# tum-pbs/PhiFlow

Measured on NVIDIA H100. Metric: smoke_plume_512^3_steps_per_sec, higher is better.
Workload: dtype f32

## Files before the change

phiflow_b200/csrc/cg_common.cuh:

```cuda
#pragma once
#include "phi_internal.cuh"

#define CG_MAX_BATCH 1024
#define CG_MAX_GRID 2048

struct CgArgs {
    DGrid g; DField pf; UnitMap um;
    const float* rhs; float* x; float* r; float* d0; float* d1;
    const float* acc;
    double* partials;
    PhiCgResult* result;
    PhiCgParams prm;
};

struct CgShared {
    double (*warp_acc)[32];
    double* sum0;
    double* sum1;
    double* delta;
    float* alpha;
    float* aprev;
    float* beta;
    float* offs;
    float* mean;
    float* tol_sq;
    float* rsq0;
    int* iters;
    int* any_cont;
    unsigned char *cont, *conv, *divg;
    float* bprev;
};

__host__ __device__ inline size_t cg_smem_bytes(int batch)
{
    const size_t b8 = ((size_t)batch + 1) / 2 * 2;
    return 2 * 32 * sizeof(double) + 3 * b8 * sizeof(double) + 8 * b8 * sizeof(float)
         + (b8 + 2) * sizeof(int) + 3 * (b8 + 16);
}

__host__ __device__ __forceinline__ CgShared cg_carve(unsigned char* base, int batch)
{
    const size_t b8 = ((size_t)batch + 1) / 2 * 2;
    CgShared sh;
    unsigned char* p = base;
    sh.warp_acc = reinterpret_cast<double (*)[32]>(p); p += 2 * 32 * sizeof(double);
    sh.sum0 = (double*)p; p += b8 * sizeof(double);
    sh.sum1 = (double*)p; p += b8 * sizeof(double);
    sh.delta = (double*)p; p += b8 * sizeof(double);
    sh.alpha = (float*)p; p += b8 * sizeof(float);
    sh.aprev = (float*)p; p += b8 * sizeof(float);
    sh.beta = (float*)p; p += b8 * sizeof(float);
    sh.offs = (float*)p; p += b8 * sizeof(float);
    sh.mean = (float*)p; p += b8 * sizeof(float);
    sh.tol_sq = (float*)p; p += b8 * sizeof(float);
    sh.rsq0 = (float*)p; p += b8 * sizeof(float);
    sh.iters = (int*)p; p += b8 * sizeof(int);
    sh.any_cont = (int*)p; p += 2 * sizeof(int);
    sh.cont = p; p += b8 + 16;
    sh.conv = p; p += b8;
    sh.divg = p; p += (b8 + 3) / 4 * 4;
    sh.bprev = (float*)p;
    return sh;
}


#ifndef CG_BLOCK_WARPS
#define CG_BLOCK_WARPS PHI_WARPS_PER_CTA
#endif

__device__ __forceinline__ void flush_partials(const CgShared& sh, double* partials, int region, int batch, int b, double a0, double a1)
{
    const int warp = threadIdx.x >> 5, lane = threadIdx.x & 31;
    a0 = warp_sum(a0); a1 = warp_sum(a1);
    if (lane == 0) { sh.warp_acc[0][warp] = a0; sh.warp_acc[1][warp] = a1; }
    __syncthreads();
    if (threadIdx.x == 0) {
        double s0 = 0, s1 = 0;
        for (int w = 0; w < (int)(blockDim.x >> 5); ++w) { s0 += sh.warp_acc[0][w]; s1 += sh.warp_acc[1][w]; }
        const size_t G = gridDim.x;
        partials[((size_t)(region * 2 + 0) * batch + b) * G + blockIdx.x] = s0;
        partials[((size_t)(region * 2 + 1) * batch + b) * G + blockIdx.x] = s1;
    }
    __syncthreads();
}

__device__ __forceinline__ void reduce_partials(const CgShared& sh, const double* partials, int region, int batch, int units_per_batch,
                                                const unsigned char* active)
{
    const int warp = threadIdx.x >> 5, lane = threadIdx.x & 31;
    const int G = gridDim.x;
    const int cnt = min(units_per_batch, G);
    for (int b = warp; b < batch; b += (int)(blockDim.x >> 5)) {
        if (active && !active[b]) continue;
        const int first = (int)(((long long)b * units_per_batch) % G);
        double s0 = 0, s1 = 0;
        for (int i = lane; i < cnt; i += 32) {
            int c = first + i; if (c >= G) c -= G;
            s0 += __ldcg(&partials[((size_t)(region * 2 + 0) * batch + b) * G + c]);
            s1 += __ldcg(&partials[((size_t)(region * 2 + 1) * batch + b) * G + c]);
        }
        s0 = warp_sum(s0); s1 = warp_sum(s1);
        if (lane == 0) { sh.sum0[b] = s0; sh.sum1[b] = s1; }
    }
    __syncthreads();
}


template <bool MASK>
__device__ __forceinline__ void cg_balance(const CgShared& sh, const PhiCgParams& prm, int b, double cells)
{
    if (MASK) { sh.mean[b] = (prm.balance_rhs && sh.sum1[b] > 0.0) ? (float)(sh.sum0[b] / sh.sum1[b]) : 0.f; sh.offs[b] = 0.f; }
    else { sh.mean[b] = prm.balance_rhs ? (float)(sh.sum0[b] / cells) : 0.f; sh.offs[b] = prm.matrix_offset * (float)sh.sum1[b]; }
}

template <bool MASK>
__device__ __forceinline__ float cg_projection_mean(const CgShared& sh, int b, double cells)
{
    return MASK ? (sh.sum1[b] > 0.0 ? (float)(sh.sum0[b] / sh.sum1[b]) : 0.f) : (float)(sh.sum0[b] / cells);
}

__device__ __forceinline__ bool cg_iteration_done(const CgShared& sh, const PhiCgParams& prm, int b, double rsq_new)
{
    sh.delta[b] = rsq_new;
    const int it = ++sh.iters[b];
    const float rsq = fabsf((float)rsq_new);
    const bool conv = rsq <= sh.tol_sq[b];
    const bool divg = !isfinite(rsq) || (rsq / sh.rsq0[b] > 1e5f && it >= 8);
    const bool cont = !conv && !divg && it < prm.max_iter;
    sh.conv[b] = conv; sh.divg[b] = divg; sh.cont[b] = cont ? 1 : 0;
    return cont;
}


__device__ __forceinline__ void cg_count_running(const CgShared& sh, int batch)
{
    __syncthreads();
    if (threadIdx.x == 0) { int any = 0; for (int b = 0; b < batch; ++b) any |= sh.cont[b]; *sh.any_cont = any; }
    __syncthreads();
}

__device__ __forceinline__ void cg_start(const CgShared& sh, const PhiCgParams& prm, int batch)
{
    for (int b = threadIdx.x; b < batch; b += blockDim.x) {
        const double d0 = sh.sum0[b], d0tol = sh.sum1[b];
        sh.delta[b] = d0;
        const float tol = fmaxf(prm.rtol * prm.rtol * (float)d0tol, prm.atol * prm.atol);
        sh.tol_sq[b] = tol; sh.rsq0[b] = (float)d0;
        const bool conv = (float)d0 <= tol;
        const bool divg = !isfinite((float)d0);
        sh.conv[b] = conv; sh.divg[b] = divg; sh.iters[b] = 0;
        sh.cont[b] = (!conv && !divg && prm.max_iter > 0) ? 1 : 0;
        sh.beta[b] = 0.f; sh.alpha[b] = 0.f; sh.aprev[b] = 0.f;
    }
    cg_count_running(sh, batch);
}

__device__ __forceinline__ void cg_write_result(const CgShared& sh, PhiCgResult* result, int batch, bool comm_ok)
{
    if (blockIdx.x != 0) return;
    for (int b = threadIdx.x; b < batch; b += blockDim.x) {
        PhiCgResult res;
        res.iterations = sh.iters[b]; res.converged = sh.conv[b]; res.diverged = comm_ok ? sh.divg[b] : -1;
        res.residual_sq = fabsf((float)sh.delta[b]); res.tol_sq = sh.tol_sq[b]; res.initial_residual_sq = sh.rsq0[b];
        result[b] = res;
    }
}
```

phiflow_b200/csrc/ring_kernels.cu:

```cuda
#include <cooperative_groups.h>
#include <type_traits>
#include "cg_common.cuh"
#include <cstdlib>
#include <cstring>
#include "launch.cuh"

namespace cg = cooperative_groups;

#define RING_CONSUMERS 256
#define RING_THREADS (RING_CONSUMERS + 32)
#define RING_MAX_STAGES 8
#define RING_G 4

struct RingCfg {
    int TY, R, pitch, nx4;
    int stage_floats;
    int ZC, nyt, nzc;
    int units_per_batch, total_units;
    int consumers;
    int groups;
    int shfl_ok;
    int split, Zm, split_t;
};

// ... 764 lines not shown
__device__ __forceinline__ bool comm_allreduce(const CommDev& cm, const CgShared& sh, int batch, unsigned long long seq)
{
    const int par = (int)(seq & 1ull);
    const size_t stride = 2 * (size_t)CG_MAX_BATCH;
    if (blockIdx.x == 0) {
        for (int q = 0; q < cm.n; ++q) {
            double* dst = cm.mbox[q] + ((size_t)par * PHI_MAX_RANKS + cm.rank) * stride;
            for (int b = threadIdx.x; b < batch; b += blockDim.x) { dst[b] = sh.sum0[b]; dst[CG_MAX_BATCH + b] = sh.sum1[b]; }
        }
        __threadfence_system();
        __syncthreads();
        if ((int)threadIdx.x < cm.n) st_release_sys(cm.flag[threadIdx.x] + par * PHI_MAX_RANKS + cm.rank, seq);
    }
    bool ok = true;
    if ((int)threadIdx.x < cm.n) {
        const unsigned long long* f = cm.flag[cm.rank] + par * PHI_MAX_RANKS + threadIdx.x;
        const long long t0 = clock64();
        while (ld_acquire_sys(f) < seq) {
            if (clock64() - t0 > 40000000000ll) { ok = false; break; }
        }
    }
    ok = __syncthreads_and(ok);
    const double* src = cm.mbox[cm.rank] + (size_t)par * PHI_MAX_RANKS * stride;
    for (int b = threadIdx.x; b < batch; b += blockDim.x) {
        double s0 = 0, s1 = 0;
        for (int q = 0; q < cm.n; ++q) {
            s0 += *(volatile const double*)(src + q * stride + b);
            s1 += *(volatile const double*)(src + q * stride + CG_MAX_BATCH + b);
        }
        sh.sum0[b] = s0; sh.sum1[b] = s1;
    }
    __syncthreads();
    return ok;
}

template <int DIM, class F>
__device__ __forceinline__ void ring_unit_cells(const RingCfg& cfg, const DGrid& g, const DField& pf, const ThreadGroups& tg,
                                                const RingUnit& u, F&& fn)
{
    if ((int)threadIdx.x >= cfg.consumers) return;
    long long plane_off = (long long)u.b * pf.sb + (long long)u.y0 * pf.sy + (DIM == 3 ? (long long)u.z0 * pf.sz : 0);
    for (int z = u.z0; z < u.z1; ++z, plane_off += pf.sz)
#pragma unroll
        for (int k = 0; k < RING_G; ++k) {
            if (tg.j[k] < 0 || u.y0 + tg.j[k] >= g.n[1]) continue;
            const int x0 = tg.eoff[k] - tg.j[k] * cfg.pitch;
            fn(plane_off + tg.goff[k], min(4, g.n[0] - x0));
        }
}

#define FUSED_GI 2
#define FUSED_GH 2
#define FUSED_TILE_BUFS 3

struct FusedGroups {
    int ti[FUSED_GI], th[FUSED_GH];
    int ei[FUSED_GI], eh[FUSED_GH];
    int gi[FUSED_GI];
    unsigned vi, vh;
};

__device__ __forceinline__ void fused_groups_init(FusedGroups& fg, const RingCfg& cfg, const DGrid& g, const DField& pf)
{
    const int lane = threadIdx.x & 31, nx = g.n[0], pitch = cfg.pitch, nx4 = cfg.nx4;
    auto edge = [&](int jj, int x0) -> int {
        const int row = jj * pitch;
        if (lane == 0) return x0 == 0 ? (pf.klo[0] == PHI_BC_PERIODIC ? row + nx - 1 : row) : row + x0 - 1;
        if (lane == 31) return x0 + 4 >= nx ? (pf.khi[0] == PHI_BC_PERIODIC ? row : row + nx - 1) : row + x0 + 4;
        return 0;
    };
    fg.vi = fg.vh = 0;
#pragma unroll
    for (int k = 0; k < FUSED_GI; ++k) {
        const int ge = threadIdx.x + k * cfg.consumers;
        const int j = ge / nx4, x0 = (ge - j * nx4) * 4;
        if (j < cfg.TY) fg.vi |= 1u << k;
        fg.ti[k] = (j + 1) * pitch + x0;
        fg.ei[k] = edge(j + 1, x0);
        fg.gi[k] = j * (int)pf.sy + x0;
    }
#pragma unroll
    for (int k = 0; k < FUSED_GH; ++k) {
        const int ge = threadIdx.x + k * cfg.consumers;
        const int h = ge / nx4, x0 = (ge - h * nx4) * 4;
        const int jj = h == 0 ? 0 : cfg.TY + 1;
        if (h < 2) fg.vh |= 1u << k;
        fg.th[k] = jj * pitch + x0;
        fg.eh[k] = edge(jj, x0);
    }
}

__device__ __forceinline__ void prod_fused_setup(ProdUnit& pu, const RingCfg& cfg, const DField& pf, const float* d, const float* dprev,
                                                 int b, int y0)
{
    const int lane = threadIdx.x & 31, TY = cfg.TY;
    const uint32_t row_bytes = (uint32_t)cfg.pitch * 4u;
    const bool mergeable = pf.sy == cfg.pitch;
    const int rows[2] = {TY + 4, TY + 2};
    const int ylo[2] = {y0 - 2, y0 - 1};
    const float* src[2] = {d, dprev};
    int cnt[2] = {0, 0};
    pu.hmask = pu.emask = 0;
#pragma unroll
    for (int it = 0; it < 4; ++it) {
        const int line = lane + 32 * it;
        pu.yoff[it] = 0; pu.base[it] = nullptr; pu.dsto[it] = 0; pu.nbytes[it] = row_bytes;
        int key = -1, yv = 0, first = 0;
#pragma unroll
        for (int arr = 0; arr < 2; ++arr) {
            if (key < 0 && line >= first && line < first + rows[arr] && src[arr]) {
                int yy = ylo[arr] + (line - first); float cv;
                phi_resolve(yy, pf, 1, cv);
                pu.yoff[it] = (long long)b * pf.sb + (long long)yy * pf.sy;
                pu.base[it] = src[arr];
                pu.dsto[it] = 4u * (uint32_t)(line * cfg.pitch);
                key = arr; yv = yy;
            }
            first += rows[arr];
        }
        cnt[0] += key == 0; cnt[1] += key == 1;
        if (prod_merge_lines(key, yv, mergeable, row_bytes, pu.nbytes[it])) {
            if (key == 0) pu.hmask |= 1u << it; else pu.emask |= 1u << it;
        }
    }
#pragma unroll
    for (int c = 0; c < 2; ++c)
#pragma unroll
        for (int o = 16; o > 0; o >>= 1) cnt[c] += __shfl_xor_sync(0xffffffffu, cnt[c], o);
    pu.tot_h = cnt[0]; pu.tot_e = cnt[1];
}

__device__ __forceinline__ float4 lds4(const float* s, int off) { return *reinterpret_cast<const float4*>(s + off); }
__device__ __forceinline__ float dot4(const float4& a, const float4& b) { return a.x * b.x + a.y * b.y + a.z * b.z + a.w * b.w; }

__device__ __forceinline__ float4 stencil7(const float4& c, float xl, float xr, const float4& ym, const float4& yp, const float4& zm, const float4& zp,
                                           float ix2, float iy2, float iz2, float cc)
{
    float4 q;
    q.x = fmaf(ix2, xl + c.y, fmaf(iy2, ym.x + yp.x, -cc * c.x));
    q.y = fmaf(ix2, c.x + c.z, fmaf(iy2, ym.y + yp.y, -cc * c.y));
    q.z = fmaf(ix2, c.y + c.w, fmaf(iy2, ym.z + yp.z, -cc * c.z));
    q.w = fmaf(ix2, c.z + xr, fmaf(iy2, ym.w + yp.w, -cc * c.w));
    q.x = fmaf(iz2, zm.x + zp.x, q.x);
    q.y = fmaf(iz2, zm.y + zp.y, q.y);
    q.z = fmaf(iz2, zm.z + zp.z, q.z);
    q.w = fmaf(iz2, zm.w + zp.w, q.w);
    return q;
}

struct FusedPass {
    const float* d; const float* dprev;
    float* dn; float* x;
    float alpha, aprev, beta, bprev;
};

__device__ __forceinline__ void ring_fused_unit(Ring& rg, const RingCfg& cfg, const DGrid& g, const DField& pf, const FusedGroups& fg,
                                                const FusedPass& P, float* tile, const RingUnit& u, float (&acc)[4])
{
    const int nz = u.z1 - u.z0;
    if ((int)threadIdx.x >= cfg.consumers) {
        ProdUnit pu;
        prod_fused_setup(pu, cfg, pf, P.d, P.dprev, u.b, u.y0);
        for (int p = 0; p < nz + 4; ++p)
            ring_produce<3>(rg, cfg, pf, pu, u.z0 - 2 + p, p >= 1 && p <= nz + 2);
        return;
    }
    const int pitch = cfg.pitch, TY = cfg.TY;
    const int pb = (TY + 4) * pitch;
    const int tsz = (TY + 2) * pitch;
    const int lane = threadIdx.x & 31;
    const float ix2 = g.inv_dx2[0], iy2 = g.inv_dx2[1], iz2 = g.inv_dx2[2];
    const float cc = 2.f * (ix2 + iy2 + iz2);
    const float alpha = P.alpha, aprev = P.aprev, beta = P.beta, bprev = P.bprev;
    const bool has_prev = P.dprev != nullptr;
    long long plane_off = (long long)u.b * pf.sb + (long long)u.y0 * pf.sy + (long long)u.z0 * pf.sz - pf.sz;

    auto dnew = [&](const float* sc, const float* sn, int o, int e, const float4& c, const float4& zm, float4& rv, float4& dp, float4& zp) {
        const float4 ym = lds4(sc, o - pitch), yp = lds4(sc, o + pitch);
        zp = lds4(sn, o);
        float xl = __shfl_up_sync(0xffffffffu, c.w, 1), xr = __shfl_down_sync(0xffffffffu, c.x, 1);
        const float ev = sc[pitch + e];
        if (lane == 0) xl = ev;
        if (lane == 31) xr = ev;
        const float4 q = stencil7(c, xl, xr, ym, yp, zm, zp, ix2, iy2, iz2, cc);
        rv = c; dp = f4_splat(0.f);
        if (has_prev) {
            dp = lds4(sc, pb + o - pitch);
            rv = make_float4(fmaf(-bprev, dp.x, c.x), fmaf(-bprev, dp.y, c.y), fmaf(-bprev, dp.z, c.z), fmaf(-bprev, dp.w, c.w));
        }
        rv.x = fmaf(-alpha, q.x, rv.x); rv.y = fmaf(-alpha, q.y, rv.y); rv.z = fmaf(-alpha, q.z, rv.z); rv.w = fmaf(-alpha, q.w, rv.w);
        return make_float4(fmaf(beta, c.x, rv.x), fmaf(beta, c.y, rv.y), fmaf(beta, c.z, rv.z), fmaf(beta, c.w, rv.w));
    };

    float4 dm[FUSED_GI], dc[FUSED_GI];
    float4 hm[FUSED_GH], hc[FUSED_GH];
    float4 n2[FUSED_GI], n1[FUSED_GI];
    float4 r1[FUSED_GI];
    float4 xv[FUSED_GI];
    SlotIt cur = rg.pos, nxt = cur; nxt.next(cfg.R);
    ring_wait_full(rg, cur); ring_wait_full(rg, nxt);
    {
        const float* s0 = ring_ptr(rg, cfg, cur);
        const float* s1 = ring_ptr(rg, cfg, nxt);
#pragma unroll
        for (int k = 0; k < FUSED_GI; ++k) {
            dm[k] = dc[k] = n2[k] = n1[k] = r1[k] = xv[k] = f4_splat(0.f);
            if (fg.vi & (1u << k)) { dm[k] = lds4(s0, pitch + fg.ti[k]); dc[k] = lds4(s1, pitch + fg.ti[k]); }
        }
#pragma unroll
        for (int k = 0; k < FUSED_GH; ++k) {
            hm[k] = hc[k] = f4_splat(0.f);
            if (fg.vh & (1u << k)) { hm[k] = lds4(s0, pitch + fg.th[k]); hc[k] = lds4(s1, pitch + fg.th[k]); }
        }
    }
    ring_release(rg, cur);
    cur = nxt; nxt.next(cfg.R);
    for (int i = 0; i < nz + 2; ++i) {
        const bool own = i >= 1 && i <= nz;
        ring_wait_full(rg, nxt);
        const float* sc = ring_ptr(rg, cfg, cur);
        const float* sn = ring_ptr(rg, cfg, nxt);
        float* tw = tile + (i % FUSED_TILE_BUFS) * tsz;
#pragma unroll
        for (int k = 0; k < FUSED_GH; ++k) {
            if (!(fg.vh & (1u << k))) continue;
            float4 rv, dp, zp;
            const float4 dv = dnew(sc, sn, pitch + fg.th[k], fg.eh[k], hc[k], hm[k], rv, dp, zp);
            *reinterpret_cast<float4*>(tw + fg.th[k]) = dv;
            hm[k] = hc[k]; hc[k] = zp;
        }
        float4 n0[FUSED_GI], r0[FUSED_GI];
        float* const dnp = P.dn + plane_off;
        float* const xp = P.x ? P.x + plane_off : nullptr;
#pragma unroll
        for (int k = 0; k < FUSED_GI; ++k) {
            n0[k] = r0[k] = f4_splat(0.f);
            if (!(fg.vi & (1u << k))) continue;
            const float4 c = dc[k];
            float4 rv, dp, zp;
            const float4 dv = dnew(sc, sn, pitch + fg.ti[k], fg.ei[k], c, dm[k], rv, dp, zp);
            *reinterpret_cast<float4*>(tw + fg.ti[k]) = dv;
            if (own) {
                *reinterpret_cast<float4*>(dnp + fg.gi[k]) = dv;
                acc[1] += dot4(rv, rv);
                if (xp) {
                    float4 x4 = xv[k];
                    x4.x += aprev * dp.x; x4.y += aprev * dp.y; x4.z += aprev * dp.z; x4.w += aprev * dp.w;
                    x4.x += alpha * c.x; x4.y += alpha * c.y; x4.z += alpha * c.z; x4.w += alpha * c.w;
                    *reinterpret_cast<float4*>(xp + fg.gi[k]) = x4;
                }
            }
            n0[k] = dv; r0[k] = rv;
            dm[k] = c; dc[k] = zp;
        }
        ring_release(rg, cur);
        if (xp && i < nz) {
#pragma unroll
            for (int k = 0; k < FUSED_GI; ++k)
                if (fg.vi & (1u << k)) xv[k] = __ldcs(reinterpret_cast<const float4*>(xp + pf.sz + fg.gi[k]));
        }
        asm volatile("bar.sync 1, %0;" ::"r"(cfg.consumers) : "memory");
        if (i >= 2) {
            const float* tp = tile + ((i - 1) % FUSED_TILE_BUFS) * tsz;
#pragma unroll
            for (int k = 0; k < FUSED_GI; ++k) {
                if (!(fg.vi & (1u << k))) continue;
                const float4 c = n1[k];
                const float4 ym = lds4(tp, fg.ti[k] - pitch), yp = lds4(tp, fg.ti[k] + pitch);
                float xl = __shfl_up_sync(0xffffffffu, c.w, 1), xr = __shfl_down_sync(0xffffffffu, c.x, 1);
                const float ev = tp[fg.ei[k]];
                if (lane == 0) xl = ev;
                if (lane == 31) xr = ev;
                const float4 q = stencil7(c, xl, xr, ym, yp, n2[k], n0[k], ix2, iy2, iz2, cc);
                acc[0] += dot4(c, q);
                acc[2] += dot4(r1[k], q);
                acc[3] += dot4(q, q);
            }
        }
#pragma unroll
        for (int k = 0; k < FUSED_GI; ++k) { n2[k] = n1[k]; n1[k] = n0[k]; r1[k] = r0[k]; }
        cur = nxt; nxt.next(cfg.R);
        plane_off += pf.sz;
    }
    ring_release(rg, cur);
    rg.pos = nxt;
    asm volatile("bar.sync 1, %0;" ::"r"(cfg.consumers) : "memory");
}

struct REpiFusedStart {
    float* d; float acc0, acc1;
    __device__ __forceinline__ void set_plane(int, int) {}
    __device__ __forceinline__ void set_acc(const float4&) {}
    __device__ __forceinline__ void operator()(long long off, const float4& c, const float4& q, int, const float4&, const float4&, const float4&)
    {
        *reinterpret_cast<float4*>(d + off) = c;
        acc0 += dot4(c, q);
        acc1 += dot4(q, q);
    }
};

template <int DIM, bool GENERIC, bool DIST, bool ADAPT, CgOp OP = CgOp::Poisson, bool FUSED = false>
__global__ void __launch_bounds__(RING_THREADS, 1)
k_cg_ring(CgRingArgs A)
{
    constexpr bool MASK = OP == CgOp::Masked;
    static_assert((OP != CgOp::Helmholtz && OP != CgOp::HelmholtzVarying) || (!DIST && !ADAPT && !FUSED),
                  "the Helmholtz operators run on the single-GPU two-sweep CG only");
    static_assert(!MASK || !ADAPT || (!DIST && !FUSED), "CG-adaptive with obstacles runs on the single-GPU two-sweep CG only");
    static_assert(!cg_op_xslot(OP) || GENERIC, "the face-minimum stencil runs on the generic consumer");
    extern __shared__ __align__(128) unsigned char smem_raw[];
    const CgArgs& a = A.a;
    const RingCfg& cfg = A.cfg;
    CgShared sh = cg_carve(smem_raw, a.g.batch);
    Ring rg;
    ring_init(rg, smem_raw + A.ring_smem_offset, cfg);
    cg::grid_group grid = cg::this_grid();
    const DGrid& g = a.g;
    const int batch = g.batch;
    const double cells = (double)g.n[0] * g.n[1] * g.n[2] * (A.cm.n > 1 ? A.cm.n : 1);
    const float coffs = a.prm.matrix_offset;
    constexpr bool adaptive = ADAPT;
    int region = 0;
    ThreadGroups tg;
    groups_init(tg, cfg, g, a.pf);
    const float* const xsrc = OP == CgOp::Masked ? a.acc : (OP == CgOp::HelmholtzVarying ? A.op.k : nullptr);

    auto sweep = [&](const unsigned char* active, auto&& body) {
        int cur_b = cfg.split ? 0 : -1; float acc0 = 0.f, acc1 = 0.f;
        RingUnit u;
        for (int k = 0; ring_next_unit<DIM>(cfg, g, k, u); ++k) {
            if (active && !active[u.b]) continue;
            if (u.b != cur_b) {
                if (cur_b >= 0) flush_partials(sh, a.partials, region, batch, cur_b, acc0, acc1);
                cur_b = u.b; acc0 = 0.f; acc1 = 0.f;
            }
            body(u, acc0, acc1);
        }
        if (cur_b >= 0) flush_partials(sh, a.partials, region, batch, cur_b, acc0, acc1);
    };
    const CommDev& cm = A.cm;
    unsigned long long seq = cm.n > 1 ? *cm.seq : 0ull;
    bool comm_ok = true;
    auto barrier_and_reduce = [&](const unsigned char* active) {
        fence_proxy_async();
        if (cm.n > 1) __threadfence_system();
        grid.sync();
        fence_proxy_async();
        reduce_partials(sh, a.partials, region, batch, cfg.split ? (int)gridDim.x : cfg.units_per_batch, active);
        region ^= 1;
        if (cm.n > 1) {
            comm_ok = comm_allreduce(cm, sh, batch, ++seq) && comm_ok;
            fence_proxy_async();
        }
    };
    const long long nzsz = (long long)g.n[2] * a.pf.sz;
    using PH = typename std::conditional<DIST, PeerHalo, NoPeerHalo>::type;
    auto peer_halo = [&](float* lo_arr, float* hi_arr) {
        PH ph;
        if constexpr (DIST) {
            ph.plo = cm.lower >= 0 ? lo_arr + nzsz : nullptr;
            ph.phi = cm.upper >= 0 ? hi_arr - nzsz : nullptr;
        }
        ph.zf = 0;
        return ph;
    };

    for (int b = threadIdx.x; b < batch; b += blockDim.x) { sh.mean[b] = 0.f; sh.offs[b] = 0.f; }
    __syncthreads();

    if (a.prm.balance_rhs || coffs != 0.f) {
        sweep(nullptr, [&](const RingUnit& u, float& acc0, float& acc1) {
            ring_unit_cells<DIM>(cfg, g, a.pf, tg, u, [&](long long off, int nvalid) {
                for (int j = 0; j < nvalid; ++j) { acc0 += a.rhs[off + j]; acc1 += MASK ? a.acc[off + j] : a.x[off + j]; }
            });
        });
        barrier_and_reduce(nullptr);
        for (int b = threadIdx.x; b < batch; b += blockDim.x) cg_balance<MASK>(sh, a.prm, b, cells);
        __syncthreads();
    }

    {
        const float* hsrc[2] = {a.x, xsrc};
        const float* esrc[2] = {a.rhs, nullptr};
        sweep(nullptr, [&](const RingUnit& u, float& acc0, float& acc1) {
            REpiResidual0<PH> epi{a.r, sh.mean[u.b], sh.offs[u.b], 0.f, 0.f, peer_halo(cm.lo_r, cm.hi_r), adaptive};
            if constexpr (OP == CgOp::Poisson) ring_process_unit<GENERIC, DIM, 1, 1>(rg, cfg, g, a.pf, tg, hsrc, esrc, 0.f, u, epi);
            else cg_op_unit<DIM, GENERIC, OP, 1, 1>(rg, A, tg, hsrc, esrc, 0.f, u, epi);
            acc0 += epi.acc0; acc1 += epi.acc1;
        });
    }
    barrier_and_reduce(nullptr);
    cg_start(sh, a.prm, batch);

    float* const D[3] = {a.d0, a.d1, A.d2};
    if constexpr (FUSED) {
        static_assert(DIM == 3 && !GENERIC && !DIST && !ADAPT && OP == CgOp::Poisson, "the one-sweep CG is 3-D, branch-free, single-GPU CG only");
        float* const tile = rg.stage0 + (size_t)cfg.R * cfg.stage_floats;
        FusedGroups fg;
        fused_groups_init(fg, cfg, g, a.pf);
        if (*sh.any_cont) {
            const float* hsrc[2] = {a.r, nullptr};
            const float* esrc[2] = {nullptr, nullptr};
            sweep(sh.cont, [&](const RingUnit& u, float& acc0, float& acc1) {
                REpiFusedStart epi{D[0], 0.f, 0.f};
                ring_process_unit<false, 3, 1, 0, true>(rg, cfg, g, a.pf, tg, hsrc, esrc, 0.f, u, epi);
                acc0 += epi.acc0; acc1 += epi.acc1;
            });
            barrier_and_reduce(sh.cont);
            for (int b = threadIdx.x; b < batch; b += blockDim.x) {
                if (!sh.cont[b]) continue;
                const double dl = sh.delta[b], dq = sh.sum0[b];
                const float al = (dq != 0.0) ? (float)(dl / dq) : 0.f;
                const double nxt = dl - 2.0 * al * dq + (double)al * al * sh.sum1[b];
                sh.alpha[b] = al;
                sh.beta[b] = (dl != 0.0) ? (float)(nxt / dl) : 0.f;
                sh.bprev[b] = 0.f;
            }
            __syncthreads();
        }
        const int upb = cfg.split ? (int)gridDim.x : cfg.units_per_batch;
        int reg = 1;
        for (int k = 0; *sh.any_cont; ++k) {
            FusedPass P;
            P.d = D[k % 3]; P.dprev = k > 0 ? D[(k + 2) % 3] : nullptr;
            P.dn = D[(k + 1) % 3]; P.x = (k & 1) ? a.x : nullptr;
            int cur_b = cfg.split ? 0 : -1;
            float acc[4] = {0.f, 0.f, 0.f, 0.f};
            RingUnit u;
            for (int j = 0; ring_next_unit<3>(cfg, g, j, u); ++j) {
                if (!sh.cont[u.b]) continue;
                if (u.b != cur_b) {
                    if (cur_b >= 0) { flush_partials(sh, a.partials, 2 * reg, batch, cur_b, acc[0], acc[1]);
                                      flush_partials(sh, a.partials, 2 * reg + 1, batch, cur_b, acc[2], acc[3]); }
                    cur_b = u.b; acc[0] = acc[1] = acc[2] = acc[3] = 0.f;
                }
                P.alpha = sh.alpha[u.b]; P.aprev = sh.aprev[u.b]; P.beta = sh.beta[u.b]; P.bprev = sh.bprev[u.b];
                ring_fused_unit(rg, cfg, g, a.pf, fg, P, tile, u, acc);
            }
            if (cur_b >= 0) { flush_partials(sh, a.partials, 2 * reg, batch, cur_b, acc[0], acc[1]);
                              flush_partials(sh, a.partials, 2 * reg + 1, batch, cur_b, acc[2], acc[3]); }
            fence_proxy_async();
            grid.sync();
            fence_proxy_async();
            reduce_partials(sh, a.partials, 2 * reg, batch, upb, sh.cont);
            for (int b = threadIdx.x; b < batch; b += blockDim.x) {
                if (!sh.cont[b]) continue;
                const double dn = sh.sum1[b], dq = sh.sum0[b];
                if (cg_iteration_done(sh, a.prm, b, dn)) {
                    sh.aprev[b] = sh.alpha[b];
                    sh.bprev[b] = sh.beta[b];
                    sh.alpha[b] = (dq != 0.0) ? (float)(dn / dq) : 0.f;
                }
            }
            __syncthreads();
            reduce_partials(sh, a.partials, 2 * reg + 1, batch, upb, sh.cont);
            for (int b = threadIdx.x; b < batch; b += blockDim.x) {
                if (!sh.cont[b]) continue;
                const double dn = sh.delta[b], al = sh.alpha[b];
                const double nxt = dn - 2.0 * al * sh.sum0[b] + al * al * sh.sum1[b];
                sh.beta[b] = (dn != 0.0) ? (float)(nxt / dn) : 0.f;
            }
            cg_count_running(sh, batch);
            reg ^= 1;
        }
        region = reg == 1 ? 2 : 0;
    }

    float* dold = a.d0; float* dnew = a.d1;
    float* lo_dnew = cm.lo_d1; float* hi_dnew = cm.hi_d1; float* lo_dold = cm.lo_d0; float* hi_dold = cm.hi_d0;
    bool x_pending = false;
    while (!FUSED && *sh.any_cont && comm_ok) {
        {
            const float* hsrc[3] = {a.r, dold, xsrc};
            const float* esrc[2] = {ADAPT ? a.r : nullptr, nullptr};
            sweep(sh.cont, [&](const RingUnit& u, float& acc0, float& acc1) {
                REpiPassA<PH, ADAPT> epi{dnew, 0.f, 0.f, peer_halo(lo_dnew, hi_dnew)};
                if constexpr (OP == CgOp::Poisson) ring_process_unit<GENERIC, DIM, 2, ADAPT ? 1 : 0>(rg, cfg, g, a.pf, tg, hsrc, esrc, sh.beta[u.b], u, epi);
                else cg_op_unit<DIM, GENERIC, OP, 2, ADAPT ? 1 : 0>(rg, A, tg, hsrc, esrc, sh.beta[u.b], u, epi);
                acc0 += epi.acc0; acc1 += epi.acc1;
            });
        }
        barrier_and_reduce(sh.cont);
        for (int b = threadIdx.x; b < batch; b += blockDim.x) {
            if (!sh.cont[b]) continue;
            sh.aprev[b] = sh.alpha[b];
            if (adaptive) {
                const double dq = sh.sum0[b];
                sh.alpha[b] = (dq != 0.0) ? (float)(sh.sum1[b] / dq) : 0.f;
                sh.delta[b] = dq;
                sh.offs[b] = 0.f;
                continue;
            }
            const double S = sh.sum1[b];
            const double dq = sh.sum0[b] + (double)coffs * S * S;
            sh.alpha[b] = (dq != 0.0) ? (float)(sh.delta[b] / dq) : 0.f;
            sh.offs[b] = coffs * (float)S;
        }
        __syncthreads();
        if (!x_pending) {
            const float* hsrc[2] = {dnew, xsrc};
            const float* esrc[3] = {a.r, nullptr, nullptr};
            sweep(sh.cont, [&](const RingUnit& u, float& acc0, float& acc1) {
                REpiPassBr<PH, ADAPT> epi{a.r, sh.alpha[u.b], ADAPT ? 0.f : sh.offs[u.b], 0.f, 0.f, peer_halo(cm.lo_r, cm.hi_r)};
                if constexpr (OP == CgOp::Poisson) ring_process_unit<GENERIC, DIM, 1, 1>(rg, cfg, g, a.pf, tg, hsrc, esrc, 0.f, u, epi);
                else cg_op_unit<DIM, GENERIC, OP, 1, 1>(rg, A, tg, hsrc, esrc, 0.f, u, epi);
                acc0 += epi.acc0; if (ADAPT) acc1 += epi.acc1;
            });
        } else {
            const float* hsrc[2] = {dnew, xsrc};
            const float* esrc[3] = {a.x, a.r, dold};
            sweep(sh.cont, [&](const RingUnit& u, float& acc0, float& acc1) {
                REpiPassB<PH, ADAPT> epi{a.x, a.r, sh.alpha[u.b], sh.aprev[u.b], ADAPT ? 0.f : sh.offs[u.b], 0.f, 0.f, peer_halo(cm.lo_r, cm.hi_r)};
                if constexpr (OP == CgOp::Poisson) ring_process_unit<GENERIC, DIM, 1, 3>(rg, cfg, g, a.pf, tg, hsrc, esrc, 0.f, u, epi);
                else cg_op_unit<DIM, GENERIC, OP, 1, 3>(rg, A, tg, hsrc, esrc, 0.f, u, epi);
                acc0 += epi.acc0; if (ADAPT) acc1 += epi.acc1;
            });
        }
        x_pending = !x_pending;
        barrier_and_reduce(sh.cont);
        for (int b = threadIdx.x; b < batch; b += blockDim.x) {
            if (!sh.cont[b]) continue;
            const double dn = sh.sum0[b];
            const double dprev = sh.delta[b];
            if (adaptive) sh.beta[b] = (dprev != 0.0) ? -(float)(sh.sum1[b] / dprev) : 0.f;
            else sh.beta[b] = (dprev != 0.0) ? (float)(dn / dprev) : 0.f;
            cg_iteration_done(sh, a.prm, b, dn);
        }
        cg_count_running(sh, batch);
        float* t = dold; dold = dnew; dnew = t;
        t = lo_dold; lo_dold = lo_dnew; lo_dnew = t;
        t = hi_dold; hi_dold = hi_dnew; hi_dnew = t;
    }

    RingUnit u;
    for (int k = 0; ring_next_unit<DIM>(cfg, g, k, u); ++k) {
        const int it = sh.iters[u.b];
        if (!(it & 1)) continue;
        const float al = sh.alpha[u.b];
        const float* dl = FUSED ? D[(it - 1) % 3] : a.d1;
        ring_unit_cells<DIM>(cfg, g, a.pf, tg, u, [&](long long off, int nvalid) {
            if (FUSED || nvalid == 4) {
                float4 xv = *reinterpret_cast<const float4*>(a.x + off);
                const float4 dv = *reinterpret_cast<const float4*>(dl + off);
                xv.x += al * dv.x; xv.y += al * dv.y; xv.z += al * dv.z; xv.w += al * dv.w;
                *reinterpret_cast<float4*>(a.x + off) = xv;
            } else for (int j = 0; j < nvalid; ++j) a.x[off + j] += al * dl[off + j];
        });
    }

    if (a.prm.project_mean) {
        sweep(nullptr, [&](const RingUnit& u, float& acc0, float& acc1) {
            ring_unit_cells<DIM>(cfg, g, a.pf, tg, u, [&](long long off, int nvalid) {
                for (int j = 0; j < nvalid; ++j) { if (MASK) { acc0 += a.x[off + j] * a.acc[off + j]; acc1 += a.acc[off + j]; } else acc0 += a.x[off + j]; }
            });
        });
        barrier_and_reduce(nullptr);
        for (int k = 0; ring_next_unit<DIM>(cfg, g, k, u); ++k) {
            const float m = cg_projection_mean<MASK>(sh, u.b, cells);
            ring_unit_cells<DIM>(cfg, g, a.pf, tg, u, [&](long long off, int nvalid) {
                for (int j = 0; j < nvalid; ++j) a.x[off + j] -= MASK ? m * a.acc[off + j] : m;
            });
        }
    }

    if (cm.n > 1 && blockIdx.x == 0 && threadIdx.x == 0) *cm.seq = seq;
    cg_write_result(sh, a.result, batch, comm_ok);
}

static const int kSmemBudget = 227 * 1024;
#define RING_UNIT_OVERHEAD 2.5

static bool ring_config(const DGrid& g, int lines_a, int lines_b, int reserve_bytes, int min_stages, int max_stages,
                        int target_units, RingCfg* out, int consumers = RING_CONSUMERS, int zhalo = 2)
{
    RingCfg c;
    c.split = 0; c.Zm = 0; c.split_t = 0;
    c.consumers = consumers;
    c.pitch = g.cext[0]; c.nx4 = g.cext[0] / 4;
    const int row_bytes = c.pitch * 4;
    int ty = g.dim == 3 ? 4 : 16;
    if (g.dim == 3) {
        const int want = 2048 / (g.cext[0] > 0 ? g.cext[0] : 1);
        ty = 1;
        while (ty * 2 <= want && ty < 16) ty *= 2;
        while (ty > 1 && ty / 2 >= g.n[1]) ty /= 2;
    }
    if (const char* e = getenv("PHICUDA_RING_TY")) { const int v = atoi(e); if (v >= 1 && v <= 32) ty = v; }
    for (;; ty /= 2) {
        if (ty < 1) return false;
        if (ty * c.nx4 > RING_G * consumers) continue;
        if (lines_a * ty + lines_b > 128) continue;
        const int stage_bytes = (lines_a * ty + lines_b) * row_bytes;
        const int r = (kSmemBudget - reserve_bytes - 128) / stage_bytes;
        if (const char* e = getenv("PHICUDA_RING_R")) { const int v = atoi(e); if (v >= min_stages && v < max_stages) max_stages = v; }
        if (r >= min_stages) { c.TY = ty; c.R = r > max_stages ? max_stages : r; c.stage_floats = stage_bytes / 4; break; }
    }
    while (g.dim == 2 && c.TY > 1 && c.TY / 2 >= g.n[1]) c.TY /= 2;
    c.groups = (c.TY * c.nx4 + consumers - 1) / consumers;
    c.shfl_ok = (c.nx4 % 32 == 0) ? 1 : 0;
    if (g.dim == 3) {
        c.nyt = (g.n[1] + c.TY - 1) / c.TY;
        const int ctas = target_units;
        double best = -1.0; int best_nzc = 1;
        const int max_nzc = g.n[2] >= 4 ? g.n[2] / 4 : 1;
        for (int nzc = 1; nzc <= max_nzc; ++nzc) {
            const int zc = (g.n[2] + nzc - 1) / nzc;
            if ((g.n[2] + zc - 1) / zc != nzc) continue;
            const long long units = (long long)c.nyt * nzc * g.batch;
            const long long rounds = (units + ctas - 1) / ctas;
            const double util = (double)units / (double)(rounds * ctas);
            const double score = util / (1.0 + (zhalo + RING_UNIT_OVERHEAD) / zc);
            if (score > best + 1e-9) { best = score; best_nzc = nzc; }
        }
        if (const char* e = getenv("PHICUDA_RING_NZC")) {
            const int v = atoi(e);
            if (v >= 1 && v <= g.n[2]) { const int zc = (g.n[2] + v - 1) / v; best_nzc = (g.n[2] + zc - 1) / zc; }
        }
        c.nzc = best_nzc; c.ZC = (g.n[2] + best_nzc - 1) / best_nzc;
        c.units_per_batch = c.nyt * c.nzc;
        c.total_units = c.units_per_batch * g.batch;
    } else {
        c.nyt = (g.n[1] + c.TY - 1) / c.TY; c.nzc = 1; c.ZC = 1;
        c.units_per_batch = c.nyt; c.total_units = c.nyt * g.batch;
    }
    *out = c;
    return true;
}

static bool ring_all_fast(const DGrid& g, const DField& f, const RingCfg& c)
{
    if (!c.shfl_ok || c.nx4 * 4 != g.n[0] || c.TY * c.nx4 != c.groups * c.consumers || g.n[1] % c.TY != 0) return false;
    for (int a = 0; a < g.dim; ++a) if (f.klo[a] == PHI_BC_CONST || f.khi[a] == PHI_BC_CONST) return false;
    return c.groups == 1 || c.groups == 2 || c.groups == 4;
}

static void note_ring_launch(int kernel, const RingCfg& c, bool generic, bool dist, bool adaptive, int grid, bool masked = false)
{
    PhiLaunchInfo li; memset(&li, 0, sizeof(li));
    li.kernel = kernel; li.generic = generic; li.dist = dist; li.adaptive = adaptive; li.masked = masked;
    li.TY = c.TY; li.stages = c.R; li.ZC = c.ZC; li.nzc = c.nzc; li.groups = c.groups; li.total_units = c.total_units; li.grid_ctas = grid; li.split = c.split;
    phi_note_launch(li);
}

int phi_launch_laplace_ring(const DGrid& g, const DField& f, const float* x, float* y, float coeff, bool axpy, cudaStream_t s)
{
    RingCfg cfg;
    const int sms = phi_sm_count();
    if (!ring_config(g, 1, 2, kSmemBudget / 2 + 1024, g.dim == 3 ? 4 : 2, 6, sms * 2, &cfg)) return -100;
    const size_t smem = 128 + (size_t)cfg.R * cfg.stage_floats * 4;
    int grid = sms * 2;
    if (grid > cfg.total_units) grid = cfg.total_units;
    cudaError_t e;
    const bool generic = !ring_all_fast(g, f, cfg);
#define LAUNCH_LAP(D, AX, GEN) do { \
        e = cudaFuncSetAttribute(k_laplace_ring<D, AX, GEN>, cudaFuncAttributeMaxDynamicSharedMemorySize, (int)smem); \
        if (e == cudaSuccess) k_laplace_ring<D, AX, GEN><<<grid, RING_THREADS, smem, s>>>(g, f, cfg, x, y, coeff); } while (0)
#define LAUNCH_LAP2(D, AX) do { if (generic) LAUNCH_LAP(D, AX, true); else LAUNCH_LAP(D, AX, false); } while (0)
    if (g.dim == 3) { if (axpy) LAUNCH_LAP2(3, true); else LAUNCH_LAP2(3, false); }
    else            { if (axpy) LAUNCH_LAP2(2, true); else LAUNCH_LAP2(2, false); }
#undef LAUNCH_LAP2
#undef LAUNCH_LAP
    if (e != cudaSuccess) return (int)e;
    note_ring_launch(PHI_KERNEL_LAPLACE_RING, cfg, generic, false, false, grid);
    return (int)cudaGetLastError();
}

static bool cg_ring_config(const DGrid& g, CgOp op, int cgs, int target_units, RingCfg* c)
{
    const bool xslot = cg_op_xslot(op);
    return ring_config(g, xslot ? 5 : 4, xslot ? 6 : 2, cgs, g.dim == 3 ? (xslot ? 3 : 4) : 2, RING_MAX_STAGES, target_units, c);
}

using CgRingKernel = void (*)(CgRingArgs);
static CgRingKernel cg_ring_kernel(CgOp op, int dim, bool generic, bool dist, bool adapt, bool fused)
{
    constexpr CgOp P = CgOp::Poisson, M = CgOp::Masked, H = CgOp::Helmholtz, V = CgOp::HelmholtzVarying;
    const bool d3 = dim == 3;
    switch (op) {
    case P:
        if (fused)
            return d3 && !generic && !dist && !adapt ? k_cg_ring<3, false, false, false, P, true> : nullptr;
        if (d3) return generic ? (dist ? (adapt ? k_cg_ring<3, true, true, true> : k_cg_ring<3, true, true, false>)
                                       : (adapt ? k_cg_ring<3, true, false, true> : k_cg_ring<3, true, false, false>))
                               : (dist ? (adapt ? k_cg_ring<3, false, true, true> : k_cg_ring<3, false, true, false>)
                                       : (adapt ? k_cg_ring<3, false, false, true> : k_cg_ring<3, false, false, false>));
        return generic ? (dist ? (adapt ? k_cg_ring<2, true, true, true> : k_cg_ring<2, true, true, false>)
                               : (adapt ? k_cg_ring<2, true, false, true> : k_cg_ring<2, true, false, false>))
                       : (dist ? (adapt ? k_cg_ring<2, false, true, true> : k_cg_ring<2, false, true, false>)
                               : (adapt ? k_cg_ring<2, false, false, true> : k_cg_ring<2, false, false, false>));
    case M:
        if (!generic || fused || (adapt && dist)) return nullptr;
        if (adapt) return d3 ? k_cg_ring<3, true, false, true, M> : k_cg_ring<2, true, false, true, M>;
        return d3 ? (dist ? k_cg_ring<3, true, true, false, M> : k_cg_ring<3, true, false, false, M>)
                  : (dist ? k_cg_ring<2, true, true, false, M> : k_cg_ring<2, true, false, false, M>);
    case H:
// ... 301 lines not shown
```

Baseline: 1.985.

## Defer solution updates in fused CG to every third iteration via recurrence

The pipelined fused CG kernel used to update x every second iteration. It now tracks a per-batch 'owed' counter and can defer the x update across two iterations. The missing direction is rebuilt from the current and previous directions plus a recomputed 7-point stencil, with coefficients derived from the stored previous alpha and beta. This cuts how often x is read and written, at the cost of an extra stencil evaluation, holding one more ring slot, and possible loss of accuracy when beta is small, which is handled by falling back to the every-other-iteration mode.

```diff
diff --git a/phiflow_b200/csrc/cg_common.cuh b/phiflow_b200/csrc/cg_common.cuh
--- a/phiflow_b200/csrc/cg_common.cuh
+++ b/phiflow_b200/csrc/cg_common.cuh
@@ -29,13 +29,16 @@
     int* any_cont;
     unsigned char *cont, *conv, *divg;
     float* bprev;
+    float* aprev2;
+    float* bprev2;
+    int* owed;
 };
 
 __host__ __device__ inline size_t cg_smem_bytes(int batch)
 {
     const size_t b8 = ((size_t)batch + 1) / 2 * 2;
-    return 2 * 32 * sizeof(double) + 3 * b8 * sizeof(double) + 8 * b8 * sizeof(float)
-         + (b8 + 2) * sizeof(int) + 3 * (b8 + 16);
+    return 2 * 32 * sizeof(double) + 3 * b8 * sizeof(double) + 10 * b8 * sizeof(float)
+         + (2 * b8 + 2) * sizeof(int) + 3 * (b8 + 16);
 }
 
 __host__ __device__ __forceinline__ CgShared cg_carve(unsigned char* base, int batch)
@@ -59,7 +62,10 @@
     sh.cont = p; p += b8 + 16;
     sh.conv = p; p += b8;
     sh.divg = p; p += (b8 + 3) / 4 * 4;
-    sh.bprev = (float*)p;
+    sh.bprev = (float*)p; p += b8 * sizeof(float);
+    sh.aprev2 = (float*)p; p += b8 * sizeof(float);
+    sh.bprev2 = (float*)p; p += b8 * sizeof(float);
+    sh.owed = (int*)p;
     return sh;
 }
 
diff --git a/phiflow_b200/csrc/ring_kernels.cu b/phiflow_b200/csrc/ring_kernels.cu
--- a/phiflow_b200/csrc/ring_kernels.cu
+++ b/phiflow_b200/csrc/ring_kernels.cu
@@ -940,8 +940,17 @@
     const float* d; const float* dprev;
     float* dn; float* x;
     float alpha, aprev, beta, bprev;
+    float xd, xdp, xq;
 };
 
+#define FUSED_XBETA_MIN 1e-2f
+
+__device__ __forceinline__ int fused_xmode(int owed, float bprev)
+{
+    return owed == 2 ? 3 : (owed == 1 && !(fabsf(bprev) >= FUSED_XBETA_MIN)) ? 2 : 0;
+}
+
+template <bool X3>
 __device__ __forceinline__ void ring_fused_unit(Ring& rg, const RingCfg& cfg, const DGrid& g, const DField& pf, const FusedGroups& fg,
                                                 const FusedPass& P, float* tile, const RingUnit& u, float (&acc)[4])
 {
@@ -985,7 +994,7 @@
     float4 n2[FUSED_GI], n1[FUSED_GI];
     float4 r1[FUSED_GI];
     float4 xv[FUSED_GI];
-    SlotIt cur = rg.pos, nxt = cur; nxt.next(cfg.R);
+    SlotIt cur = rg.pos, nxt = cur, prv = cur; nxt.next(cfg.R);
     ring_wait_full(rg, cur); ring_wait_full(rg, nxt);
     {
         const float* s0 = ring_ptr(rg, cfg, cur);
@@ -1031,7 +1040,21 @@
             if (own) {
                 *reinterpret_cast<float4*>(dnp + fg.gi[k]) = dv;
                 acc[1] += dot4(rv, rv);
-                if (xp) {
+                if constexpr (X3) {
+                    const int od = pb + fg.ti[k];
+                    const float4 ym = lds4(sc, od - pitch), yp = lds4(sc, od + pitch), zpp = lds4(sn, od);
+                    float xl = __shfl_up_sync(0xffffffffu, dp.w, 1), xr = __shfl_down_sync(0xffffffffu, dp.x, 1);
+                    const float ev = sc[pb + fg.ei[k]];
+                    if (lane == 0) xl = ev;
+                    if (lane == 31) xr = ev;
+                    const float4 q = stencil7(dp, xl, xr, ym, yp, lds4(ring_ptr(rg, cfg, prv), od), zpp, ix2, iy2, iz2, cc);
+                    float4 x4 = xv[k];
+                    x4.x = fmaf(P.xq, q.x, fmaf(P.xdp, dp.x, fmaf(P.xd, c.x, x4.x)));
+                    x4.y = fmaf(P.xq, q.y, fmaf(P.xdp, dp.y, fmaf(P.xd, c.y, x4.y)));
+                    x4.z = fmaf(P.xq, q.z, fmaf(P.xdp, dp.z, fmaf(P.xd, c.z, x4.z)));
+                    x4.w = fmaf(P.xq, q.w, fmaf(P.xdp, dp.w, fmaf(P.xd, c.w, x4.w)));
+                    *reinterpret_cast<float4*>(xp + fg.gi[k]) = x4;
+                } else if (xp) {
                     float4 x4 = xv[k];
                     x4.x += aprev * dp.x; x4.y += aprev * dp.y; x4.z += aprev * dp.z; x4.w += aprev * dp.w;
                     x4.x += alpha * c.x; x4.y += alpha * c.y; x4.z += alpha * c.z; x4.w += alpha * c.w;
@@ -1041,7 +1064,8 @@
             n0[k] = dv; r0[k] = rv;
             dm[k] = c; dc[k] = zp;
         }
-        ring_release(rg, cur);
+        if constexpr (X3) { if (i > 0) ring_release(rg, prv); prv = cur; }
+        else ring_release(rg, cur);
         if (xp && i < nz) {
 #pragma unroll
             for (int k = 0; k < FUSED_GI; ++k)
@@ -1070,6 +1094,7 @@
         cur = nxt; nxt.next(cfg.R);
         plane_off += pf.sz;
     }
+    if constexpr (X3) ring_release(rg, prv);
     ring_release(rg, cur);
     rg.pos = nxt;
     asm volatile("bar.sync 1, %0;" ::"r"(cfg.consumers) : "memory");
@@ -1186,6 +1211,8 @@
         float* const tile = rg.stage0 + (size_t)cfg.R * cfg.stage_floats;
         FusedGroups fg;
         fused_groups_init(fg, cfg, g, a.pf);
+        for (int b = threadIdx.x; b < batch; b += blockDim.x) sh.owed[b] = 0;
+        __syncthreads();
         if (*sh.any_cont) {
             const float* hsrc[2] = {a.r, nullptr};
             const float* esrc[2] = {nullptr, nullptr};
@@ -1211,7 +1238,7 @@
         for (int k = 0; *sh.any_cont; ++k) {
             FusedPass P;
             P.d = D[k % 3]; P.dprev = k > 0 ? D[(k + 2) % 3] : nullptr;
-            P.dn = D[(k + 1) % 3]; P.x = (k & 1) ? a.x : nullptr;
+            P.dn = D[(k + 1) % 3];
             int cur_b = cfg.split ? 0 : -1;
             float acc[4] = {0.f, 0.f, 0.f, 0.f};
             RingUnit u;
@@ -1223,7 +1250,15 @@
                     cur_b = u.b; acc[0] = acc[1] = acc[2] = acc[3] = 0.f;
                 }
                 P.alpha = sh.alpha[u.b]; P.aprev = sh.aprev[u.b]; P.beta = sh.beta[u.b]; P.bprev = sh.bprev[u.b];
-                ring_fused_unit(rg, cfg, g, a.pf, fg, P, tile, u, acc);
+                const int xm = fused_xmode(sh.owed[u.b], P.bprev);
+                P.x = xm ? a.x : nullptr;
+                if (xm == 3) {
+                    const double gam = (double)sh.aprev2[u.b] / sh.bprev2[u.b];
+                    P.xd = (float)(P.alpha - gam);
+                    P.xdp = (float)(P.aprev + gam * (1.0 + P.bprev));
+                    P.xq = (float)(-gam * P.aprev);
+                    ring_fused_unit<true>(rg, cfg, g, a.pf, fg, P, tile, u, acc);
+                } else ring_fused_unit<false>(rg, cfg, g, a.pf, fg, P, tile, u, acc);
             }
             if (cur_b >= 0) { flush_partials(sh, a.partials, 2 * reg, batch, cur_b, acc[0], acc[1]);
                               flush_partials(sh, a.partials, 2 * reg + 1, batch, cur_b, acc[2], acc[3]); }
@@ -1234,7 +1269,11 @@
             for (int b = threadIdx.x; b < batch; b += blockDim.x) {
                 if (!sh.cont[b]) continue;
                 const double dn = sh.sum1[b], dq = sh.sum0[b];
+                const int ow = sh.owed[b];
+                sh.owed[b] = fused_xmode(ow, sh.bprev[b]) ? 0 : ow + 1;
                 if (cg_iteration_done(sh, a.prm, b, dn)) {
+                    sh.aprev2[b] = sh.aprev[b];
+                    sh.bprev2[b] = sh.bprev[b];
                     sh.aprev[b] = sh.alpha[b];
                     sh.bprev[b] = sh.beta[b];
                     sh.alpha[b] = (dq != 0.0) ? (float)(dn / dq) : 0.f;
@@ -1323,12 +1362,19 @@
     RingUnit u;
     for (int k = 0; ring_next_unit<DIM>(cfg, g, k, u); ++k) {
         const int it = sh.iters[u.b];
-        if (!(it & 1)) continue;
+        const int owe = FUSED ? sh.owed[u.b] : (it & 1);
+        if (!owe) continue;
         const float al = sh.alpha[u.b];
         const float* dl = FUSED ? D[(it - 1) % 3] : a.d1;
+        const float ap = sh.aprev[u.b];
+        const float* dl2 = D[(it + 1) % 3];
         ring_unit_cells<DIM>(cfg, g, a.pf, tg, u, [&](long long off, int nvalid) {
             if (FUSED || nvalid == 4) {
                 float4 xv = *reinterpret_cast<const float4*>(a.x + off);
+                if (FUSED && owe == 2) {
+                    const float4 dp = *reinterpret_cast<const float4*>(dl2 + off);
+                    xv.x += ap * dp.x; xv.y += ap * dp.y; xv.z += ap * dp.z; xv.w += ap * dp.w;
+                }
                 const float4 dv = *reinterpret_cast<const float4*>(dl + off);
                 xv.x += al * dv.x; xv.y += al * dv.y; xv.z += al * dv.z; xv.w += al * dv.w;
                 *reinterpret_cast<float4*>(a.x + off) = xv;
```

Measured after the change: 2.098 (median of 6 runs). 5.7% higher.
